# bevanda/Learning-Based-MPC

Hardware: AMD Instinct MI355X
Metric: QP-steps/s (whole node) at N=20 Moore-Greitzer; KKT-residual vs MATLAB ref (higher is better)
Workload: dtype f64; 1 GPU; C2: MG LMPC (F1) N=20, 616-row terminal set, batch 1024 per GPU, fp64; batch_per_gpu=1024, horizon=20, parallelism=dp1, streams=1

## Files before the change

### learning-based-mpc_amd/csrc/bqp_ocp.hip

```cpp
#include <hip/hip_runtime.h>
#include <math.h>
#include <stdint.h>
#include <stdlib.h>

#include <type_traits>

#include "bqp_internal.h"
#include "bqp_lanes.h"
#include "bqp_wave.h"

namespace bqp {

#ifdef BQP_F32
typedef float real;
typedef float2 real2;
#define BQP_SFX _f32
namespace sp {
#else
typedef double real;
typedef double2 real2;
#define BQP_SFX
namespace dp {
#endif
#define BQP_CAT2(a, b) a##b
#define BQP_CAT(a, b) BQP_CAT2(a, b)

#define WAVE 64
#ifdef BQP_F32
#define BQP_LNG_OK 0
#else
#define BQP_LNG_OK 1
#endif
#ifdef BQP_F32
#define PIV_FLOOR 1e-7
#else
#define PIV_FLOOR 1e-14
#endif
#define MU_BLOWUP 1e6
#ifdef BQP_F32
#define FEAS_GUARD 1e-6
#define BQP_POLISH 0
#else
#define FEAS_GUARD 1e-8
#define BQP_POLISH 1
#endif
#ifndef BQP_EXP_NOROW
#define BQP_EXP_NOROW 0
#endif
#ifndef BQP_EXP_NOSTAGE
#define BQP_EXP_NOSTAGE 0
#endif
#define TAU_FAST_AFF 0.99
#define TAU_FAST_MU 1e-6
#define TAU_FAST 0.99999
#define TAU_FAST_END 0.99999
#define TAU_FAST_MIN 0.995
#define CMAX_K 100.0
#define SOC_ALPHA 0.1
#define DEG_POLISH 1e-10
#define POL_RHO 2e6
#define POL_ROUNDS 8
#define POL_PASS 3
#define POL_CG 40
#define POL_CG_SING 1e-2
#define POL_STAG 0.5

__device__ __forceinline__ double frcp(double t) {
    double r = __builtin_amdgcn_rcp(t);
    double e = __builtin_fma(-t, r, 1.0);
    r = __builtin_fma(r, e, r);
    e = __builtin_fma(-t, r, 1.0);
    return __builtin_fma(r, e, r);
}
__device__ __forceinline__ float frcp(float t) {
    float r = __builtin_amdgcn_rcpf(t);
    return __builtin_fmaf(r, __builtin_fmaf(-t, r, 1.0f), r);
}

__device__ __forceinline__ int opq(int v) {
    asm volatile("" : "+v"(v));
    return v;
}
__device__ __forceinline__ int opq_s(int v) {
    asm volatile("" : "+s"(v));
    return v;
}

__device__ __forceinline__ double fmar(double a, double b, double c) { return __builtin_fma(a, b, c); }
__device__ __forceinline__ float fmar(float a, float b, float c) { return __builtin_fmaf(a, b, c); }
constexpr bool SWEEP_DPP_FMAC = sizeof(real) == 8;
#ifndef BQP_SWEEP_ROWS
#define BQP_SWEEP_ROWS 1
#endif
#ifdef BQP_F32
#define MADD(acc, a, b) acc = fmar((a), (b), (acc))
#else
#define MADD(acc, a, b) acc += (a) * (b)
#endif

template <int N>
__device__ __forceinline__ bool chol_small(const real (&M)[N][N], real (&L)[N][N]) {
    bool ok = true;
    real d0 = M[0][0];
    if (!(d0 > PIV_FLOOR * M[0][0])) d0 = PIV_FLOOR * M[0][0];
    ok = ok && (d0 > 0.0);
    if constexpr (N == 2) {
        const real r0 = frcp(d0);
        const real l10 = M[1][0] * r0;
        real d1 = M[1][1] - l10 * M[1][0];
        if (!(d1 > PIV_FLOOR * M[1][1])) d1 = PIV_FLOOR * M[1][1];
        ok = ok && (d1 > 0.0);
        L[0][0] = r0;
        L[0][1] = 0.0;
        L[1][0] = l10;
        L[1][1] = frcp(d1);
    } else {
        L[0][0] = sqrt(d0);
    }
    return ok;
}
template <int N>
__device__ __forceinline__ void chol_solve_small(const real* L, real (&b)[N]) {
    if constexpr (N == 2) {
        const real w1 = (b[1] - L[2] * b[0]) * L[3];
        b[0] = b[0] * L[0] - L[2] * w1;
        b[1] = w1;
    } else {
        b[0] = b[0] * L[0];
    }
}

__host__ __device__ constexpr int pk_len(int NS) { return NS * (NS + 1) / 2; }
__host__ __device__ constexpr int pk_stride(int NS) {
    return (((pk_len(NS) + 1) & ~1) % 4 == 0) ? ((pk_len(NS) + 1) & ~1) + 2 : ((pk_len(NS) + 1) & ~1);
}
__host__ __device__ constexpr int pk_idx(int NS, int i, int j) {
    return i <= j ? i * NS - i * (i - 1) / 2 + (j - i) : j * NS - j * (j - 1) / 2 + (i - j);
}

__host__ __device__ constexpr int stg_len(int NX, int NU) { return NX * NX + NX * NU + NX; }
__host__ __device__ constexpr int stg_stride(int NX, int NU) { return stg_len(NX, NU) | 1; }

enum : int {
    X_CNT = 0,
    X_BSR,
    X_FEASB,
    X_CS,
    X_STOP,
    X_ALPHA,
    X_CMAX,
    X_FEASOK,
    X_FLAG,
    X_RHO,
    X_TF,
    X_DEG,
    X_PVA,
    X_PVIOL,
    X_PLNEG,
    X_PLMX,
    X_PCHG,
    X_PDEC,
    X_CGD,
    X_NXCH = 20
};
constexpr int X_NEXT = X_PVA;
static_assert(X_PVIOL == X_PVA + 1, "X_NEXT + 1 must be a polish-only slot");
constexpr int X_RSS = X_PLNEG;
constexpr int X_PEN = X_PLMX;

struct QpLds {
    int P, K, Lr, L0, AB, xs, xu, qt_xpi, rs, ru, re, pv, wv, bw, qu, fv, dsv, duv, dsc, duc, Dx, FD,
        blam, ebox, bnd, gpp, gpe, prp, hp, rp, xch, Fi, Hi, total;
    __host__ __device__ __forceinline__ static QpLds make(int N, int NX, int NU, int NP, int mpad, bool fpi = false,
                                          bool lng = false, bool hpsh = false, bool bndsh = false,
                                          bool hinst = false, bool stg = false) {
// ... 10 lines not shown
        o.qt_xpi = c; c += (N + 1) * NS;
        o.rs = c;     c += (N + 1) * NS;
        o.ru = c;     c += (N + 1) * NU;
        o.re = c;     c += lng ? 0 : (N + 1) * NS;
        o.pv = c;     c += (N + 1) * NS;
        o.wv = c;     c += (N + 1) * NS;
        o.bw = c;     c += (N + 1) * NU;
        o.qu = c;     c += (N + 1) * NU;
        if (lng) {
            o.fv = o.qt_xpi;
        } else {
            o.fv = c; c += (N + 1) * NS;
        }
        o.dsv = c;    c += (N + 1) * NS;
        o.duv = c;    c += (N + 1) * NU;
        o.dsc = c;    c += (N + 1) * NS;
        o.duc = c;    c += (N + 1) * NU;
        o.Dx = c;     c += (N + 1) * NV;
        o.FD = c;     c += NV * NV;
        o.blam = c;   c += (N + 1) * NB * (lng ? 1 : 2);
        o.ebox = c;   c += (N + 1) * NB * (lng ? 1 : 2);
        o.bnd = c;    c += bndsh ? 0 : (N + 1) * NB * 2;
        o.gpp = c;    c += NV;
        o.gpe = c;    c += NV;
        o.prp = c;    c += mpad;
        o.hp = c;     c += hpsh ? 0 : mpad;
        o.rp = c;     c += lng ? 0 : mpad;
        o.xch = c;    c += X_NXCH;
        o.Fi = c;     c += fpi ? NV * mpad : 0;
        o.Hi = c;     c += (hinst && !lng) ? (N + 1) * (NV * NV + 1) : 0;
        o.total = (c + 1) & ~1;
        return o;
    }
};

__host__ __device__ constexpr int hand_stage_w(int NS, int NU) { return 2 * NS + NU; }
__host__ __device__ constexpr int hand_rows_off(int N, int NS, int NU) {
    return ((N + 1) * hand_stage_w(NS, NU) + 63) & ~63;
}
#ifdef BQP_F32
#define BQP_HAND_IN 0
#define BQP_HAND_OUT 1
#else
#define BQP_HAND_IN 1
#define BQP_HAND_OUT 0
#endif
template <bool LONG, bool POL>
__device__ __forceinline__ bool hand_warm(const OcpKernelArgs& a, int inst) {
    return BQP_HAND_IN && LONG && a.hand_in && (a.hand_flag[inst] == 1 || a.hand_flag[inst] == 0) &&
           !(POL && a.pol_need[inst] == 2);
}

#ifdef BQP_STAMPS
#define STAMP(id)                                                          \
    do {                                                                   \
        __builtin_amdgcn_s_waitcnt(0);                                     \
        const unsigned long long _t = __builtin_amdgcn_s_memtime();        \
        st_acc[id] += _t - st_last;                                        \
        st_last = _t;                                                      \
    } while (0)
#define STAMP_DECL                                                         \
    unsigned long long st_last = __builtin_amdgcn_s_memtime();             \
    unsigned long long st_acc[16];                                         \
    _Pragma("unroll") for (int i_ = 0; i_ < 16; ++i_) st_acc[i_] = 0
#define STAMP_STORE(base)                                                  \
    do {                                                                   \
        if (lane == 0 && a.stamps) {                                       \
            _Pragma("unroll") for (int i_ = 0; i_ < 16; ++i_)              \
                a.stamps[(int64_t)inst * 32 + (base) + i_] = (double)st_acc[i_]; \
        }                                                                  \
    } while (0)
#elif defined(BQP_ISA_ONLY_MG10) || defined(BQP_ISA_ONLY_DI) || defined(BQP_ISA_ONLY_MG_LNG)
#define STAMP(id) asm volatile(";BQP_PHASE " #id)
#define STAMP_DECL do { } while (0)
#define STAMP_STORE(base) do { } while (0)
#else
#define STAMP(id) do { } while (0)
#define STAMP_DECL do { } while (0)
#define STAMP_STORE(base) do { } while (0)
#endif

#if defined(BQP_STAMPS) && defined(BQP_STAMPS_SPLIT)
#define STAMP_SPLIT(id) STAMP(id)
#else
#define STAMP_SPLIT(id) do { } while (0)
#endif

#define BARRIER() __syncthreads()
#define ROW_FENCE(q) do { if ((q) & 1) __builtin_amdgcn_sched_barrier(0); } while (0)

template <int NX, int NU, int NP, int SPL, bool POL, int G, bool STG = false, bool SOFT = false>
__device__ __forceinline__ void stage_wave(const OcpKernelArgs& a, real* W, const QpLds& L,
                                           const real* Hs, int lane_w, int inst, int pslot) {
    const int lane = lane_w;
    constexpr bool PC = POL && BQP_POLISH && !BQP_EXP_NOSTAGE;
    constexpr int NS = NX + NP;
    constexpr int NV = NS + NU;
    constexpr int NB = NX + NU;
    static_assert(G == 1 || (SPL == 1 && lanes::compiled(NS, NU, G)), "lane groups: short horizons only");
    static_assert(!STG || (G == 1 && sizeof(real) == 8), "per-stage models: fp64, G = 1");
    static_assert(!STG || SWEEP_DPP_FMAC, "per-stage models: the sweeps' DPP form only");
    static_assert(!SOFT || (STG && !POL), "soft state bounds: per-stage-model solve kernels only");
    constexpr int ES = lanes::entries_per_lane(NS, G);
    const int N = a.N, kp = a.kp, hstride = a.hstride;
    auto stage_of = [&](int ln, int j) __attribute__((always_inline)) -> int {
        if constexpr (G > 1) return lanes::stage_lane(ln, N, G).k;
        else return ln + WAVE * j;
    };
    real* X = W + L.xch;
    STAMP_DECL;
    constexpr bool LNG = BQP_LNG_OK && SPL == 2;
#define BQP_HK(k) const real* Hk = Hs + (k) * hstride; \
    const double* Hkg = (a.H_inst ? a.H_inst + (int64_t)inst * (N + 1) * hstride : a.H) + (int64_t)(k) * hstride
#define BQP_HV(idx) (LNG ? (real)Hkg[idx] : Hk[idx])
    real* Pgl = LNG ? (real*)a.Pg + (int64_t)pslot * (N + 1) * pk_stride(NS) : nullptr;
    if (!LNG && a.H_inst) {
        real* Hl = W + L.Hi;
        const double* Hg = a.H_inst + (int64_t)inst * (N + 1) * hstride;
        for (int i = lane; i < (N + 1) * hstride; i += WAVE) Hl[i] = (real)Hg[i];
        wave_sync();
        Hs = Hl;
    }

    const double* Ag = STG ? a.A + (int64_t)inst * a.sA : nullptr;
    const double* Bg = STG ? a.B + (int64_t)inst * a.sB : nullptr;
    const double* cg = (STG && a.c) ? a.c + (int64_t)inst * a.sc : nullptr;
    constexpr int MW = stg_len(NX, NU), MST = stg_stride(NX, NU);
    if constexpr (STG) {
        if constexpr (!LNG) {
            for (int t = lane; t < N * MW; t += WAVE) {
                const int k = t / MW, e = t - k * MW;
                int kg = k;
                if constexpr (SOFT) { if (a.one_model) kg = 0; }
                real v;
                if (e < NX * NX) v = Ag[(int64_t)kg * (NX * NX) + e];
                else if (e < NX * NX + NX * NU) v = Bg[(int64_t)kg * (NX * NU) + (e - NX * NX)];
                else v = cg ? cg[(int64_t)kg * NX + (e - NX * NX - NX * NU)] : 0.0;
                W[L.AB + k * MST + e] = v;
            }
        }
    } else {
        const double* A = a.A + (int64_t)inst * a.sA;
        const double* B = a.B + (int64_t)inst * a.sB;
        if (lane < NS * NS) {
            const int i = lane / NS, j = lane % NS;
            W[L.AB + lane] = (i < NX && j < NX) ? A[j * NX + i] : (i == j ? 1.0 : 0.0);
        }
        if (lane < NS * NU) {
            const int i = lane / NU, j = lane % NU;
            W[L.AB + NS * NS + lane] = (i < NX) ? B[j * NX + i] : 0.0;
        }
        if (lane < NS) W[L.AB + NS * NS + NS * NU + lane] = (lane < NX && a.c) ? a.c[(int64_t)inst * a.sc + lane] : 0.0;
    }
    wave_sync();
    auto mdl = [&](int k, int e) __attribute__((always_inline)) -> real {
        const int km = k < N ? k : N - 1;
        if constexpr (LNG) {
            int kg = km;
            if constexpr (SOFT) { if (a.one_model) kg = 0; }
            if (e < NX * NX) return (real)Ag[(int64_t)kg * (NX * NX) + e];
            if (e < NX * NX + NX * NU) return (real)Bg[(int64_t)kg * (NX * NU) + (e - NX * NX)];
            return cg ? (real)cg[(int64_t)kg * NX + (e - NX * NX - NX * NU)] : real(0);
        } else {
            return W[L.AB + km * MST + e];
        }
    };
    auto Abar = [&](int k, int i, int j) __attribute__((always_inline)) -> real {
        if constexpr (STG) {
// ... 159 lines not shown
#pragma unroll
                    for (int c = 0; c < NS; ++c) MADD(acc, Abar(k, i, c), s[j][c]);
#pragma unroll
                    for (int c = 0; c < NU; ++c) MADD(acc, Bbar(k, i, c), u[j][c]);
                    if constexpr (!LNG) W[L.re + k * NS + i] = acc;
                    fe = fmax(fe, fabs(acc));
                }
            }
        }
        feasA = wmax(fe);
        gsA = wmax(gs);
    };

    bool rez = false;
    auto re_at = [&](int j, int k, int i) __attribute__((always_inline)) -> real {
        if constexpr (PC) { if (rez) return real(0); }
        real acc = cb(k, i) - W[L.xs + (k + 1) * NS + i];
#pragma unroll
        for (int c = 0; c < NS; ++c) MADD(acc, Abar(k, i, c), s[j][c]);
#pragma unroll
        for (int c = 0; c < NU; ++c) MADD(acc, Bbar(k, i, c), u[j][c]);
        return acc;
    };

    auto combine = [&]() __attribute__((always_inline)) -> real {
        const int lane = opq(lane_w);
        real gpp[NV];
#pragma unroll
        for (int c = 0; c < NV; ++c) gpp[c] = W[L.gpp + c];
        real st = 0;
#pragma unroll
        for (int j = 0; j < SPL; ++j) {
            const int k = stage_of(lane, j);
            if (k > N) continue;
            real r[NS], ru[NU];
#pragma unroll
            for (int i = 0; i < NS; ++i) r[i] = W[L.rs + k * NS + i];
#pragma unroll
            for (int i = 0; i < NU; ++i) ru[i] = W[L.ru + k * NU + i];
#pragma unroll
            for (int i = 0; i < NX; ++i) {
                if constexpr (LNG) {
                    r[i] += W[L.blam + k * NB + i];
                } else {
                    r[i] += W[L.blam + (k * NB + i) * 2];
                    r[i] -= W[L.blam + (k * NB + i) * 2 + 1];
                }
            }
#pragma unroll
            for (int i = 0; i < NU; ++i) {
                if constexpr (LNG) {
                    ru[i] += W[L.blam + k * NB + NX + i];
                } else {
                    ru[i] += W[L.blam + (k * NB + NX + i) * 2];
                    ru[i] -= W[L.blam + (k * NB + NX + i) * 2 + 1];
                }
            }
            if (k == kp) {
#pragma unroll
                for (int i = 0; i < NS; ++i) r[i] += gpp[i];
                if (kp < N) {
#pragma unroll
                    for (int i = 0; i < NU; ++i) ru[i] += gpp[NS + i];
                }
            }
            if (k == 0) {
#pragma unroll
                for (int i = 0; i < NX; ++i) r[i] = 0.0;
            }
#pragma unroll
            for (int i = 0; i < NS; ++i) { st = fmax(st, fabs(r[i])); W[L.rs + k * NS + i] = r[i]; }
#pragma unroll
            for (int i = 0; i < NU; ++i) { st = fmax(st, fabs(ru[i])); W[L.ru + k * NU + i] = ru[i]; }
        }
        wave_sync();
        return wmax(st);
    };

    constexpr int PST = pk_stride(NS);
    constexpr int NPK = pk_len(NS);
    constexpr int NUT = NU * (NU + 1) / 2;
    constexpr int VAL = 1 + 2 * NU + NUT;
    constexpr int VPL = (VAL + 3) / 4;
    static_assert(4 * NPK <= WAVE, "one quad per packed entry of P");
    const int fq = lane >> 2, fql = lane & 3;
    const bool fquad = fq < NPK;
    int ie = 0, je = 0;
    {
        int e = 0;
#pragma unroll
        for (int i = 0; i < NS; ++i)
#pragma unroll
            for (int j = i; j < NS; ++j, ++e)
                if (e == fq) { ie = i; je = j; }
    }
    auto vrc = [&](int v, int& r, int& c) __attribute__((always_inline)) {
        if (v == 0) { r = ie; c = je; }
        else if (v <= NU) { r = ie; c = NS + v - 1; }
        else if (v <= 2 * NU) { r = je; c = NS + v - NU - 1; }
        else {
            int t = v - 2 * NU - 1, x = 0;
#pragma unroll
            for (int xx = 0; xx < NU; ++xx) if (t >= NU - xx) { t -= NU - xx; x = xx + 1; } else break;
            r = NS + x; c = NS + x + t;
        }
    };
    real cf[STG ? 1 : VPL][STG ? 1 : NPK];
    int vr[VPL], vc[VPL];
    int fr[VPL], fc[VPL];
#pragma unroll
    for (int t = 0; t < VPL; ++t) {
        const int v = fql + 4 * t;
        int r = 0, c = 0;
        if (v < VAL) vrc(v, r, c);
        vr[t] = r; vc[t] = c;
        if constexpr (STG) {
            fr[t] = r < NX ? r * NX : (r >= NS ? (NX + r - NS) * NX : -1);
            fc[t] = c < NX ? c * NX : (c >= NS ? (NX + c - NS) * NX : -1);
        } else {
            auto Fab = [&](int a_, int r_) __attribute__((always_inline)) -> real {
                return r_ < NS ? Abar(0, a_, r_) : Bbar(0, a_, r_ - NS);
            };
            int m = 0;
#pragma unroll
            for (int a_ = 0; a_ < NS; ++a_)
#pragma unroll
                for (int b = a_; b < NS; ++b, ++m) {
                    real x = Fab(a_, r) * Fab(b, c);
                    if (a_ != b) x = fmar(Fab(b, r), Fab(a_, c), x);
                    cf[t][m] = (v < VAL) ? x : real(0);
                }
        }
    }
    struct HNoModel {};
    struct HModel { real mr[VPL][NX], mc[VPL][NX]; };
    struct HRaw : std::conditional_t<STG, HModel, HNoModel> { real h[VPL], d[VPL]; };
    auto load_h = [&](int k, HRaw& o) __attribute__((always_inline)) {
        BQP_HK(k);
#pragma unroll
        for (int t = 0; t < VPL; ++t) {
            o.h[t] = BQP_HV(vr[t] * NV + vc[t]);
            o.d[t] = W[L.Dx + k * NV + vr[t]];
            if constexpr (STG) {
#pragma unroll
                for (int a_ = 0; a_ < NX; ++a_) {
                    const real xr = mdl(k, (fr[t] < 0 ? 0 : fr[t]) + a_);
                    const real xc = mdl(k, (fc[t] < 0 ? 0 : fc[t]) + a_);
                    o.mr[t][a_] = fr[t] < 0 ? real(0) : xr;
                    o.mc[t][a_] = fc[t] < 0 ? real(0) : xc;
                }
            }
        }
    };
    auto cf_at = [&](const HRaw& o, int t, int a_, int b) __attribute__((always_inline)) -> real {
        if constexpr (STG) {
            auto Fr = [&](int i) __attribute__((always_inline)) -> real {
                return i < NX ? o.mr[t][i < NX ? i : 0] : (vr[t] == i ? real(1) : real(0));
            };
            auto Fc = [&](int i) __attribute__((always_inline)) -> real {
                return i < NX ? o.mc[t][i < NX ? i : 0] : (vc[t] == i ? real(1) : real(0));
            };
            real x = Fr(a_) * Fc(b);
            if (a_ != b) x = fmar(Fr(b), Fc(a_), x);
            return (fql + 4 * t < VAL) ? x : real(0);
        } else {
            return real(0);
        }
    };
    auto ht = [&](int k, const HRaw& o, int t) __attribute__((always_inline)) -> real {
        real v = o.h[t] + (vr[t] == vc[t] ? o.d[t] : real(0));
        if (k == kp) v += W[L.FD + vr[t] * NV + vc[t]];
        return v;
    };
    real pu[PST];
    auto read_p = [&](int k) __attribute__((always_inline)) {
        wave_sync();
        const real2* src = reinterpret_cast<const real2*>(W + L.P + (LNG ? (k & 1) : k) * PST);
#pragma unroll
        for (int q = 0; q < PST / 2; ++q) {
            const real2 t2 = src[q];
            pu[2 * q] = t2.x;
            pu[2 * q + 1] = t2.y;
        }
    };
    auto Pm = [&](int a_, int b_) __attribute__((always_inline)) -> real { return pu[pk_idx(NS, a_, b_)]; };
    auto factor = [&]() __attribute__((always_inline)) -> bool {
        HRaw raw, nxt;
        {
            load_h(N, raw);
            const real v0 = ht(N, raw, 0);
            if (fquad && fql == 0) {
                W[L.P + (LNG ? (N & 1) : N) * PST + fq] = v0;
                if constexpr (LNG) Pgl[N * PST + fq] = v0;
            }
        }
        read_p(N);
        bool ok = true;
        auto fstage = [&](int k, const HRaw& raw) __attribute__((always_inline)) {
            real mv[VPL];
#pragma unroll
            for (int t = 0; t < VPL; ++t) {
                real sp0 = 0, sp1 = 0, sp2 = 0, sp3 = 0;
                if constexpr (STG) {
                    int m = 0;
#pragma unroll
                    for (int a_ = 0; a_ < NS; ++a_)
#pragma unroll
                        for (int b = a_; b < NS; ++b, ++m) {
                            const real cm = cf_at(raw, t, a_, b);
                            if ((m & 3) == 0) sp0 = fmar(cm, pu[m], sp0);
                            if ((m & 3) == 1) sp1 = fmar(cm, pu[m], sp1);
                            if ((m & 3) == 2) sp2 = fmar(cm, pu[m], sp2);
                            if ((m & 3) == 3) sp3 = fmar(cm, pu[m], sp3);
                        }
                } else {
#pragma unroll
                for (int m = 0; m < NPK; ++m) {
                    if ((m & 3) == 0) sp0 = fmar(cf[t][m], pu[m], sp0);
                    if ((m & 3) == 1) sp1 = fmar(cf[t][m], pu[m], sp1);
                    if ((m & 3) == 2) sp2 = fmar(cf[t][m], pu[m], sp2);
                    if ((m & 3) == 3) sp3 = fmar(cf[t][m], pu[m], sp3);
                }
                }
                mv[t] = ht(k, raw, t) + ((sp0 + sp1) + (sp2 + sp3));
            }
            real g[VAL];
#pragma unroll
            for (int v = 0; v < VAL; ++v) {
                const int s = v & 3;
                const real src = mv[v >> 2];
                g[v] = (s == 0) ? dpp_mov0<0x00>(src)
                     : (s == 1) ? dpp_mov0<0x55>(src)
                     : (s == 2) ? dpp_mov0<0xAA>(src)
                                : dpp_mov0<0xFF>(src);
            }
            real pv, Kc[NU], Lf[NU * NU];
            if constexpr (NU == 1) {
                ok = ok && (g[3] > 0.0);
                const real rinv = frcp(g[3]);
                Lf[0] = rinv;
                pv = fmar(-(g[1] * rinv), g[2], g[0]);
                Kc[0] = -(g[2] * rinv);
            } else {
                real Mu[NU][NU], Lc[NU][NU];
                {
                    int t = 2 * NU + 1;
#pragma unroll
                    for (int x = 0; x < NU; ++x)
#pragma unroll
                        for (int y = x; y < NU; ++y, ++t) { Mu[x][y] = g[t]; Mu[y][x] = g[t]; }
                }
                ok = chol_small<NU>(Mu, Lc) && ok;
#pragma unroll
                for (int x = 0; x < NU; ++x)
#pragma unroll
                    for (int y = 0; y < NU; ++y) Lf[x * NU + y] = Lc[x][y];
                real y[NU];
#pragma unroll
                for (int x = 0; x < NU; ++x) y[x] = g[1 + NU + x];
                chol_solve_small<NU>(Lf, y);
                real acc = g[1] * y[0];
#pragma unroll
                for (int x = 1; x < NU; ++x) acc = fmar(g[1 + x], y[x], acc);
                pv = g[0] - acc;
#pragma unroll
                for (int x = 0; x < NU; ++x) Kc[x] = -y[x];
            }
            if (fquad && fql == 0) {
                W[L.P + (LNG ? (k & 1) : k) * PST + fq] = pv;
                if constexpr (LNG) Pgl[k * PST + fq] = pv;
                if (ie == je) {
#pragma unroll
                    for (int x = 0; x < NU; ++x) W[L.K + k * NU * NS + x * NS + je] = Kc[x];
                }
                if (fq == 0) {
#pragma unroll
                    for (int x = 0; x < NU * NU; ++x) W[L.Lr + k * NU * NU + x] = Lf[x];
                }
            }
            read_p(k);
        };
        if constexpr (LNG) {
            HRaw r0, r1, r2;
            load_h(N - 1, r0);
            if (N >= 2) load_h(N - 2, r1);
            for (int k = N - 1; k >= 0; k -= 3) {
                if (k >= 2) load_h(k - 2, r2);
                fstage(k, r0);
                if (k < 1) break;
                if (k >= 3) load_h(k - 3, r0);
                fstage(k - 1, r1);
                if (k < 2) break;
                if (k >= 4) load_h(k - 4, r1);
                fstage(k - 2, r2);
            }
        } else {
            load_h(N - 1, raw);
            for (int k = N - 1; k >= 0; --k) {
                if (k > 0) load_h(k - 1, nxt);
                fstage(k, raw);
                raw = nxt;
            }
        }
        real Pt[NP][NP], L0[NP][NP];
#pragma unroll
        for (int x = 0; x < NP; ++x)
#pragma unroll
            for (int y = 0; y < NP; ++y) Pt[x][y] = Pm(NX + x, NX + y);
        if constexpr (NP == 1) {
            ok = ok && (Pt[0][0] > 0.0);
            L0[0][0] = 1.0 / Pt[0][0];
        } else {
            ok = chol_small<NP>(Pt, L0) && ok;
        }
        if (lane == 0) {
#pragma unroll
            for (int x = 0; x < NP; ++x)
#pragma unroll
                for (int y = 0; y < NP; ++y) W[L.L0 + x * NP + y] = L0[x][y];
        }
        if constexpr (LNG) asm volatile("s_waitcnt vmcnt(0)" ::: "memory");
        wave_sync();
        return ok;
    };
    auto load_pk = [&](int k, real* pk) __attribute__((always_inline)) {
        if constexpr (LNG) {
            const real* src = Pgl + k * PST;
#pragma unroll
            for (int e = 0; e < NPK; ++e) pk[e] = __hip_atomic_load(src + e, __ATOMIC_RELAXED, __HIP_MEMORY_SCOPE_AGENT);
        } else {
#pragma unroll
            for (int e = 0; e < NPK; ++e) pk[e] = W[L.P + k * PST + e];
        }
    };

    auto prep_iter = [&]() __attribute__((always_inline)) {
        const int lane = opq(lane_w);
        if constexpr (G > 1) {
            const lanes::StageLane sl = lanes::stage_lane(lane, N, G);
            const int k = sl.k;
            if (k < N) {
                const real* Pn = W + L.P + (k + 1) * PST;
                const real* Kk = W + L.K + k * NU * NS;
                real rek[NS], wk[NS];
#pragma unroll
                for (int c = 0; c < NS; ++c) rek[c] = W[L.re + k * NS + c];
#pragma unroll
                for (int i = 0; i < NS; ++i) {
                    real v = 0.0;
#pragma unroll
                    for (int c = 0; c < NS; ++c) MADD(v, Pn[pk_idx(NS, i, c)], rek[c]);
                    wk[i] = v;
                }
#pragma unroll
                for (int x = 0; x < NU; ++x) {
                    real v = 0.0;
#pragma unroll
                    for (int c = 0; c < NS; ++c) MADD(v, Bbar(k, c, x), wk[c]);
                    W[L.bw + k * NU + x] = v;
                }
#pragma unroll
                for (int t = 0; t < ES; ++t) {
                    const int i = lanes::entry(NS, G, sl.g, t);
                    real v = 0.0;
#pragma unroll
                    for (int c = 0; c < NS; ++c) {
                        real ph = Abar(k, c, i);
#pragma unroll
                        for (int x = 0; x < NU; ++x) MADD(ph, Bbar(k, c, x), Kk[x * NS + i]);
                        MADD(v, ph, wk[c]);
                    }
                    W[L.wv + k * NS + i] = v;
                }
            }
            return;
        }
#pragma unroll
        for (int j = 0; j < SPL; ++j) {
            const int k = stage_of(lane, j);
            if (k < N) {
                real Pn_[LNG ? PST : 1];
                const real* Pn = W + L.P + (k + 1) * PST;
                if constexpr (LNG) { load_pk(k + 1, Pn_); Pn = Pn_; }
                const real* Kk = W + L.K + k * NU * NS;
                real rek[NS], wk[NS];
#pragma unroll
                for (int c = 0; c < NS; ++c) rek[c] = LNG ? re_at(j, k, c) : W[L.re + k * NS + c];
#pragma unroll
                for (int i = 0; i < NS; ++i) {
                    real v = 0.0;
#pragma unroll
// ... 597 lines not shown
            for (int i = 0; i < NS; ++i) MADD(s[j][i], al, dsk[i]);
            if (k < N) {
#pragma unroll
                for (int i = 0; i < NU; ++i) MADD(u[j][i], al, W[idu + k * NU + i]);
            }
        }
    };

    real feasA = 0, gsA = 0;
    real minv, bscale;
    int flag = 0, it0 = 0;
    if (hand_warm<SPL == 2, POL>(a, inst)) {
        const float* hb = a.hand_in + (int64_t)inst * a.hand_stride;
        constexpr int SW = hand_stage_w(NS, NU);
#pragma unroll
        for (int j = 0; j < SPL; ++j) {
            const int k = stage_of(lane, j);
            if (k > N) continue;
#pragma unroll
            for (int i = 0; i < NS; ++i) {
                s[j][i] = (k == 0 && i < NX) ? s[j][i] : (real)hb[k * SW + i];
                pi[j][i] = (real)hb[k * SW + NS + i];
            }
#pragma unroll
            for (int i = 0; i < NU; ++i) u[j][i] = (k < N) ? (real)hb[k * SW + 2 * NS + i] : 0.0;
        }
        write_state();
        stage_partials(feasA, gsA);
        BARRIER();
        minv = 1.0 / fmax(X[X_CNT], 1.0);
        bscale = fmax(x0max, X[X_BSR]);
        it0 = a.hand_it[inst];
    } else {
        write_state();
        stage_partials(feasA, gsA);
        BARRIER();
        minv = 1.0 / fmax(X[X_CNT], 1.0);
        bscale = fmax(x0max, X[X_BSR]);
        combine();
        if (!factor()) flag = -8;
        prep_iter();
        BARRIER();
        solve(L.dsv, L.duv);
        update_stage(1.0, L.dsv, L.duv);
        BARRIER();
        BARRIER();
        write_state();
        stage_partials(feasA, gsA);
    }

    int it = 0;
    real mu = 0.0, mu_min = INFINITY, stat = 0.0, feas = 0.0, feq = 0.0, fin = 0.0;
    const int max_iter = a.max_iter;
    for (it = 0;; ++it) {
        BARRIER();
        STAMP(0);
        stat = combine();
        if constexpr (SOFT) stat = fmax(stat, X[X_RSS]);
        STAMP(1);
        STAMP(2);
        feq = feasA;
        fin = X[X_FEASB];
        feas = fmax(feq, fin);
        mu = X[X_CS] * minv;
        bool stop = false;
        if (flag != 0) {
            stop = true;
        } else if (stat <= a.tol_stat * (1.0 + gsA) && feas <= a.tol_feas * (1.0 + bscale) &&
                   mu <= a.tol_comp && (!BQP_POLISH || X[X_CMAX] <= CMAX_K * a.tol_comp)) {
            flag = 1; stop = true;
#ifdef BQP_F32
        } else if (mu <= a.tol_comp && feas <= a.tol_feas * (1.0 + bscale) && isfinite(stat)) {
            flag = 1; stop = true;
#endif
        } else if (!(isfinite(stat) && isfinite(feas) && isfinite(mu))) {
            flag = -8; stop = true;
        } else if (mu > MU_BLOWUP * mu_min && feas > FEAS_GUARD * (1.0 + bscale)) {
            flag = -2; stop = true;
        } else {
            mu_min = fmin(mu_min, mu);
            if (it == max_iter) stop = true;
        }
        if (!stop && !factor()) { flag = -8; stop = true; }
        if (!stop) prep_iter();
        STAMP(3);
        if (lane == 0) {
            X[X_STOP] = stop ? 1.0 : 0.0;
            X[X_FEASOK] = (feas <= FEAS_GUARD * (1.0 + bscale)) ? 1.0 : 0.0;
            X[X_FLAG] = (real)flag;
            if constexpr (PC) {
                X[X_RHO] = POL_RHO * (1.0 + gsA);
                X[X_TF] = 1e-12 * (1.0 + bscale);
            }
        }
        BARRIER();
        STAMP(4);
        if (stop) break;
        solve(L.dsv, L.duv);
        STAMP(5);
        BARRIER();
        BARRIER();
        STAMP(6);
        solve(L.dsc, L.duc);
        STAMP(7);
        BARRIER();
        dual_dir(L.dsc);
        BARRIER();
        STAMP(8);
        const real al = X[X_ALPHA];
        update_stage_dir(al, L.dsc, L.duc);
        write_state();
        stage_partials(feasA, gsA);
        STAMP(9);
    }

    real polished = 0.0;
    bool pi_kept = false;
    if constexpr (PC) {
        BARRIER();
        const bool dopol = a.polish > 0 && flag != -2 &&
                           (flag != 1 || (a.polish > 1 && X[X_DEG] > DEG_POLISH)) && isfinite(gsA);
        if (dopol) {
            STAMP(15);
#pragma unroll
            for (int j = 0; j < SPL; ++j) {
                const int k = lane + WAVE * j;
                if (a.pi_out && k >= 1 && k <= N) {
                    double* po = a.pi_out + ((int64_t)inst * N + (k - 1)) * NX;
#pragma unroll
                    for (int i = 0; i < NX; ++i) po[i] = pi[j][i];
                }
                if (k <= N) {
#pragma unroll
                    for (int i = 0; i < NS; ++i) W[L.dsv + k * NS + i] = s[j][i];
#pragma unroll
                    for (int i = 0; i < NU; ++i) W[L.duv + k * NU + i] = (k < N) ? u[j][i] : 0.0;
                }
            }
            const real tf = 1e-12 * (1.0 + bscale);
            int rd = 0, pass = 0, m = 0, dec = 0;
            real pst = 0.0;
            auto zero_stage_res = [&]() __attribute__((always_inline)) {
#pragma unroll
                for (int j = 0; j < SPL; ++j) {
                    const int k = stage_of(lane, j);
                    if (k > N) continue;
#pragma unroll
                    for (int i = 0; i < NS; ++i) {
                        W[L.rs + k * NS + i] = 0.0;
                        if constexpr (!LNG) W[L.re + k * NS + i] = 0.0;
                    }
#pragma unroll
                    for (int i = 0; i < NU; ++i) W[L.ru + k * NU + i] = 0.0;
                }
                wave_sync();
            };
            for (;;) {
                stage_partials(feasA, gsA);
                BARRIER();
                BARRIER();
                pst = combine();
                const real va = X[X_PVA];
                if (m != 1) {
                    dec = factor() ? 0 : 3;
                    pass = 0;
                } else {
                    const bool pok = isfinite(pst) && pst <= a.tol_stat * (1.0 + gsA) && va <= tf;
                    if (!pok && pass + 1 < POL_PASS) {
// ... 1871 lines not shown
```

### learning-based-mpc_amd/csrc/bqp_wave.h

```cpp
#pragma once
#include <hip/hip_runtime.h>
#include <math.h>

namespace bqp {

__device__ __forceinline__ void wave_sync() {
    __builtin_amdgcn_fence(__ATOMIC_RELEASE, "wavefront");
    __builtin_amdgcn_wave_barrier();
    __builtin_amdgcn_fence(__ATOMIC_ACQUIRE, "wavefront");
}

template <int CTRL, int ROWM>
__device__ __forceinline__ double dpp_mov(double old, double v) {
    const int2 o = __builtin_bit_cast(int2, old);
    const int2 x = __builtin_bit_cast(int2, v);
    int2 r;
    r.x = __builtin_amdgcn_update_dpp(o.x, x.x, CTRL, ROWM, 0xf, false);
    r.y = __builtin_amdgcn_update_dpp(o.y, x.y, CTRL, ROWM, 0xf, false);
    return __builtin_bit_cast(double, r);
}
template <int CTRL>
__device__ __forceinline__ double dpp_mov0(double v) {
    const int2 x = __builtin_bit_cast(int2, v);
    int2 r;
// ... 84 lines not shown
    v += dpp_mov<0x143, 0xc>(0.0f, v);
    return lane63(v);
}
__device__ __forceinline__ float wmax(float v) {
    v = fmaxf(v, dpp_mov<0xB1, 0xf>(-INFINITY, v));
    v = fmaxf(v, dpp_mov<0x4E, 0xf>(-INFINITY, v));
    v = fmaxf(v, dpp_mov<0x141, 0xf>(-INFINITY, v));
    v = fmaxf(v, dpp_mov<0x140, 0xf>(-INFINITY, v));
    v = fmaxf(v, dpp_mov<0x142, 0xa>(-INFINITY, v));
    v = fmaxf(v, dpp_mov<0x143, 0xc>(-INFINITY, v));
    return lane63(v);
}
__device__ __forceinline__ float wmin(float v) { return -wmax(-v); }
__device__ __forceinline__ float rl(float v, int src) {
    return __builtin_bit_cast(float, __builtin_amdgcn_readlane(__builtin_bit_cast(int, v), src));
}

template <int C>
__device__ __forceinline__ double rbc(double v) {
    return __builtin_amdgcn_update_dpp(0.0, v, 0x150 + C, 0xf, 0xf, true);
}
template <int C>
__device__ __forceinline__ float rbc(float v) {
    return __builtin_bit_cast(float, __builtin_amdgcn_update_dpp(0, __builtin_bit_cast(int, v),
                                                                 0x150 + C, 0xf, 0xf, true));
}
template <int Q>
__device__ __forceinline__ double xrow_bcast(double v) {
    double a = v, b = v;
    pl16_swap(a, b);
    double c = (Q & 1) ? b : a, d = c;
    pl32_swap(c, d);
    return (Q >> 1) ? d : c;
}

template <int C, int NC, typename T>
__device__ __forceinline__ void rbc_all(T v, T (&p)[NC]) {
    p[C] = rbc<C>(v);
    if constexpr (C + 1 < NC) rbc_all<C + 1, NC>(v, p);
}

template <int C, bool FRESH = false, typename T>
__device__ __forceinline__ void fmac_rbc(T& acc, T v, T ph) {
    static_assert(sizeof(T) == 8, "fmac_rbc: fp64 only (the fp32 sweeps keep rbc + plain products)");
    static_assert(C >= 0 && C < 16, "fmac_rbc: lane of a 16-lane row");
    if constexpr (FRESH)
        asm("s_nop 1\n\t"
            "v_fmac_f64_dpp %0, %1, %2 row_newbcast:%3 row_mask:0xf bank_mask:0xf bound_ctrl:1"
            : "+v"(acc) : "v"(v), "v"(ph), "n"(C));
    else
        asm("v_fmac_f64_dpp %0, %1, %2 row_newbcast:%3 row_mask:0xf bank_mask:0xf bound_ctrl:1"
            : "+v"(acc) : "v"(v), "v"(ph), "n"(C));
}
template <int C, int NC, typename T>
__device__ __forceinline__ void fmac_rbc_seq(T& acc, T v, const T (&ph)[NC]) {
    fmac_rbc<C, C == 0>(acc, v, ph[C]);
    if constexpr (C + 1 < NC) fmac_rbc_seq<C + 1, NC>(acc, v, ph);
}
#define BQP_FMAC_RBC(OP, C) \
    "v_fmac_f64_dpp %0, %2, %" #OP " row_newbcast:" #C " row_mask:0xf bank_mask:0xf bound_ctrl:1\n\t"
#define BQP_CHAIN_HEAD \
    "v_mov_b64 %0, %1\n\t" \
    "s_nop 0\n\t"
template <int NC, typename T>
__device__ __forceinline__ T fmac_rbc_chain(T q, T v, const T (&ph)[NC]) {
    static_assert(sizeof(T) == 8, "fmac_rbc_chain: fp64 only");
    T acc;
    if constexpr (NC == 4) {
        asm(BQP_CHAIN_HEAD BQP_FMAC_RBC(3, 0) BQP_FMAC_RBC(4, 1) BQP_FMAC_RBC(5, 2) BQP_FMAC_RBC(6, 3)
            : "=&v"(acc) : "v"(q), "v"(v), "v"(ph[0]), "v"(ph[1]), "v"(ph[2]), "v"(ph[3]));
    } else if constexpr (NC == 5) {
        asm(BQP_CHAIN_HEAD BQP_FMAC_RBC(3, 0) BQP_FMAC_RBC(4, 1) BQP_FMAC_RBC(5, 2) BQP_FMAC_RBC(6, 3)
            BQP_FMAC_RBC(7, 4)
            : "=&v"(acc) : "v"(q), "v"(v), "v"(ph[0]), "v"(ph[1]), "v"(ph[2]), "v"(ph[3]), "v"(ph[4]));
    } else {
        acc = q;
        fmac_rbc_seq<0, NC>(acc, v, ph);
    }
    return acc;
}
#undef BQP_CHAIN_HEAD
#undef BQP_FMAC_RBC

template <int CTRL, typename T, int KI, int KO>
__device__ __forceinline__ void tsum_step(const T (&in)[KI], T (&out)[KO], bool hi) {
#pragma unroll
    for (int p = 0; p < KO; ++p) {
        const T a = in[2 * p];
        const T b = (2 * p + 1 < KI) ? in[2 * p + 1] : T(0);
        const T keep = hi ? b : a;
        const T send = hi ? a : b;
        out[p] = keep + dpp_mov0<CTRL>(send);
    }
}
template <typename T, int K>
__device__ __forceinline__ T wsum_t(const T (&v)[K], int lane) {
    static_assert(K >= 2 && K <= 32, "wsum_t: 2..32 values");
    constexpr int K1 = (K + 1) / 2, K2 = (K1 + 1) / 2, K3 = (K2 + 1) / 2, K4 = (K3 + 1) / 2;
    T w1[K1], w2[K2], w3[K3], w4[K4];
    tsum_step<0xB1>(v, w1, (lane & 1) != 0);
    tsum_step<0x4E>(w1, w2, (lane & 2) != 0);
    tsum_step<0x124>(w2, w3, (lane & 4) != 0);
    tsum_step<0x128>(w3, w4, (lane & 8) != 0);
    T a = w4[0], b = T(0);
    if constexpr (K4 > 1) b = w4[K4 - 1];
    pl16_swap(a, b);
    T c = a + b, d = c;
    pl32_swap(c, d);
    return c + d;
}

}
```

Before: 2.808 million QP-steps/s.

## Factor Riccati stage with row-layout packed P held in registers via DPP broadcasts

Remaps the factor's lane assignment so each 16-lane row holds one packed entry of P per lane, with the four rows carrying different value groups. The P-times-coefficient dot product now uses v_fmac_f64_dpp row_newbcast from the register-resident P, and results are gathered with permlane swaps. This removes the LDS write/read round trip of P at each stage along with its wave syncs. It also inlines the 2x2 Cholesky solve and moves a timing stamp. The new path is limited to fp64, SPL==1 and NPK<=16, and relies on inline asm and permlane ops that must be correct for this layout.

```diff
diff --git a/learning-based-mpc_amd/csrc/bqp_ocp.hip b/learning-based-mpc_amd/csrc/bqp_ocp.hip
--- a/learning-based-mpc_amd/csrc/bqp_ocp.hip
+++ b/learning-based-mpc_amd/csrc/bqp_ocp.hip
@@ -91,6 +91,9 @@
 constexpr bool SWEEP_DPP_FMAC = sizeof(real) == 8;
 #ifndef BQP_SWEEP_ROWS
 #define BQP_SWEEP_ROWS 1
+#endif
+#ifndef BQP_FACTOR_ROWS
+#define BQP_FACTOR_ROWS 1
 #endif
 #ifdef BQP_F32
 #define MADD(acc, a, b) acc = fmar((a), (b), (acc))
@@ -267,8 +270,10 @@
 
 #if defined(BQP_STAMPS) && defined(BQP_STAMPS_SPLIT)
 #define STAMP_SPLIT(id) STAMP(id)
+#define STAMP_PLAIN(id) do { } while (0)
 #else
 #define STAMP_SPLIT(id) do { } while (0)
+#define STAMP_PLAIN(id) STAMP(id)
 #endif
 
 #define BARRIER() __syncthreads()
@@ -594,8 +599,12 @@
     constexpr int NUT = NU * (NU + 1) / 2;
     constexpr int VAL = 1 + 2 * NU + NUT;
     constexpr int VPL = (VAL + 3) / 4;
+    constexpr bool FACTOR_ROWS = BQP_FACTOR_ROWS && sizeof(real) == 8 && SPL == 1;
     static_assert(4 * NPK <= WAVE, "one quad per packed entry of P");
-    const int fq = lane >> 2, fql = lane & 3;
+    static_assert(!FACTOR_ROWS || NPK <= 16, "FACTOR_ROWS: one packed entry of P per lane of a row");
+    static_assert(!FACTOR_ROWS || NP <= 2, "FACTOR_ROWS: the theta block's entries are taken one by one");
+    const int fq = FACTOR_ROWS ? ((lane & 15) < NPK ? (lane & 15) : NPK - 1) : lane >> 2;
+    const int fql = FACTOR_ROWS ? lane >> 4 : lane & 3;
     const bool fquad = fq < NPK;
     int ie = 0, je = 0;
     {
@@ -698,22 +707,42 @@
     auto Pm = [&](int a_, int b_) __attribute__((always_inline)) -> real { return pu[pk_idx(NS, a_, b_)]; };
     auto factor = [&]() __attribute__((always_inline)) -> bool {
         HRaw raw, nxt;
+        real pl = 0;
         {
             load_h(N, raw);
             const real v0 = ht(N, raw, 0);
+            if constexpr (FACTOR_ROWS) {
+                pl = xrow_bcast<0>(v0);
+                W[L.P + N * PST + fq] = pl;
+            } else {
             if (fquad && fql == 0) {
                 W[L.P + (LNG ? (N & 1) : N) * PST + fq] = v0;
                 if constexpr (LNG) Pgl[N * PST + fq] = v0;
             }
-        }
-        read_p(N);
+            }
+        }
+        if constexpr (!FACTOR_ROWS) read_p(N);
         bool ok = true;
         auto fstage = [&](int k, const HRaw& raw) __attribute__((always_inline)) {
             real mv[VPL];
 #pragma unroll
             for (int t = 0; t < VPL; ++t) {
                 real sp0 = 0, sp1 = 0, sp2 = 0, sp3 = 0;
-                if constexpr (STG) {
+                if constexpr (FACTOR_ROWS) {
+                    real sp[4];
+                    if constexpr (STG) {
+                        real cm[NPK];
+                        int m = 0;
+#pragma unroll
+                        for (int a_ = 0; a_ < NS; ++a_)
+#pragma unroll
+                            for (int b = a_; b < NS; ++b, ++m) cm[m] = cf_at(raw, t, a_, b);
+                        fmac_rbc_dot4(sp, pl, cm);
+                    } else {
+                        fmac_rbc_dot4(sp, pl, cf[t]);
+                    }
+                    sp0 = sp[0]; sp1 = sp[1]; sp2 = sp[2]; sp3 = sp[3];
+                } else if constexpr (STG) {
                     int m = 0;
 #pragma unroll
                     for (int a_ = 0; a_ < NS; ++a_)
@@ -737,6 +766,15 @@
                 mv[t] = ht(k, raw, t) + ((sp0 + sp1) + (sp2 + sp3));
             }
             real g[VAL];
+            if constexpr (FACTOR_ROWS) {
+#pragma unroll
+                for (int t = 0; t < VPL; ++t) {
+                    real g4[4];
+                    xrow_gather(mv[t], g4);
+#pragma unroll
+                    for (int s = 0; s < 4; ++s) if (4 * t + s < VAL) g[4 * t + s] = g4[s];
+                }
+            } else {
 #pragma unroll
             for (int v = 0; v < VAL; ++v) {
                 const int s = v & 3;
@@ -745,6 +783,7 @@
                      : (s == 1) ? dpp_mov0<0x55>(src)
                      : (s == 2) ? dpp_mov0<0xAA>(src)
                                 : dpp_mov0<0xFF>(src);
+            }
             }
             real pv, Kc[NU], Lf[NU * NU];
             if constexpr (NU == 1) {
@@ -770,13 +809,28 @@
                 real y[NU];
 #pragma unroll
                 for (int x = 0; x < NU; ++x) y[x] = g[1 + NU + x];
-                chol_solve_small<NU>(Lf, y);
+                if constexpr (FACTOR_ROWS && NU == 2) {
+                    const real w1 = (y[1] - Lf[2] * y[0]) * Lf[3];
+                    y[0] = fmar(y[0], Lf[0], -(Lf[2] * w1));
+                    y[1] = w1;
+                } else {
+                    chol_solve_small<NU>(Lf, y);
+                }
                 real acc = g[1] * y[0];
 #pragma unroll
                 for (int x = 1; x < NU; ++x) acc = fmar(g[1 + x], y[x], acc);
                 pv = g[0] - acc;
 #pragma unroll
                 for (int x = 0; x < NU; ++x) Kc[x] = -y[x];
+            }
+            if constexpr (FACTOR_ROWS) {
+                W[L.P + k * PST + fq] = pv;
+#pragma unroll
+                for (int x = 0; x < NU; ++x) W[L.K + k * NU * NS + x * NS + je] = Kc[x];
+#pragma unroll
+                for (int x = 0; x < NU * NU; ++x) W[L.Lr + k * NU * NU + x] = Lf[x];
+                pl = pv;
+                return;
             }
             if (fquad && fql == 0) {
                 W[L.P + (LNG ? (k & 1) : k) * PST + fq] = pv;
@@ -818,7 +872,14 @@
 #pragma unroll
         for (int x = 0; x < NP; ++x)
 #pragma unroll
-            for (int y = 0; y < NP; ++y) Pt[x][y] = Pm(NX + x, NX + y);
+            for (int y = 0; y < NP; ++y) Pt[x][y] = FACTOR_ROWS ? real(0) : Pm(NX + x, NX + y);
+        if constexpr (FACTOR_ROWS) {
+            Pt[0][0] = rbc<pk_idx(NS, NX, NX)>(pl);
+            if constexpr (NP == 2) {
+                Pt[0][1] = Pt[1][0] = rbc<pk_idx(NS, NX, NX + 1)>(pl);
+                Pt[1][1] = rbc<pk_idx(NS, NX + 1, NX + 1)>(pl);
+            }
+        }
         if constexpr (NP == 1) {
             ok = ok && (Pt[0][0] > 0.0);
             L0[0][0] = 1.0 / Pt[0][0];
@@ -1582,8 +1643,9 @@
             if (it == max_iter) stop = true;
         }
         if (!stop && !factor()) { flag = -8; stop = true; }
+        STAMP_SPLIT(3);
         if (!stop) prep_iter();
-        STAMP(3);
+        STAMP_PLAIN(3);
         if (lane == 0) {
             X[X_STOP] = stop ? 1.0 : 0.0;
             X[X_FEASOK] = (feas <= FEAS_GUARD * (1.0 + bscale)) ? 1.0 : 0.0;
diff --git a/learning-based-mpc_amd/csrc/bqp_wave.h b/learning-based-mpc_amd/csrc/bqp_wave.h
--- a/learning-based-mpc_amd/csrc/bqp_wave.h
+++ b/learning-based-mpc_amd/csrc/bqp_wave.h
@@ -190,6 +190,55 @@
 #undef BQP_CHAIN_HEAD
 #undef BQP_FMAC_RBC
 
+#define BQP_DOT4_ZERO \
+    "v_mov_b64 %0, 0\n\tv_mov_b64 %1, 0\n\tv_mov_b64 %2, 0\n\tv_mov_b64 %3, 0\n\t"
+#define BQP_DOT4_FMAC(ACC, OP, C) \
+    "v_fmac_f64_dpp %" #ACC ", %4, %" #OP " row_newbcast:" #C " row_mask:0xf bank_mask:0xf bound_ctrl:1\n\t"
+template <int M, int NC, typename T>
+__device__ __forceinline__ void fmac_rbc_dot4_seq(T (&s)[4], T v, const T (&c)[NC]) {
+    fmac_rbc<M, (M < 4)>(s[M & 3], v, c[M]);
+    if constexpr (M + 1 < NC) fmac_rbc_dot4_seq<M + 1, NC>(s, v, c);
+}
+template <int NC, typename T>
+__device__ __forceinline__ void fmac_rbc_dot4(T (&s)[4], T v, const T (&c)[NC]) {
+    static_assert(sizeof(T) == 8, "fmac_rbc_dot4: fp64 only");
+    static_assert(NC >= 4 && NC <= 16, "fmac_rbc_dot4: one entry per lane of a 16-lane row");
+    if constexpr (NC == 10) {
+        asm(BQP_DOT4_ZERO
+            BQP_DOT4_FMAC(0, 5, 0) BQP_DOT4_FMAC(1, 6, 1) BQP_DOT4_FMAC(2, 7, 2) BQP_DOT4_FMAC(3, 8, 3)
+            BQP_DOT4_FMAC(0, 9, 4) BQP_DOT4_FMAC(1, 10, 5) BQP_DOT4_FMAC(2, 11, 6) BQP_DOT4_FMAC(3, 12, 7)
+            BQP_DOT4_FMAC(0, 13, 8) BQP_DOT4_FMAC(1, 14, 9)
+            : "=&v"(s[0]), "=&v"(s[1]), "=&v"(s[2]), "=&v"(s[3])
+            : "v"(v), "v"(c[0]), "v"(c[1]), "v"(c[2]), "v"(c[3]), "v"(c[4]), "v"(c[5]), "v"(c[6]),
+              "v"(c[7]), "v"(c[8]), "v"(c[9]));
+    } else if constexpr (NC == 15) {
+        asm(BQP_DOT4_ZERO
+            BQP_DOT4_FMAC(0, 5, 0) BQP_DOT4_FMAC(1, 6, 1) BQP_DOT4_FMAC(2, 7, 2) BQP_DOT4_FMAC(3, 8, 3)
+            BQP_DOT4_FMAC(0, 9, 4) BQP_DOT4_FMAC(1, 10, 5) BQP_DOT4_FMAC(2, 11, 6) BQP_DOT4_FMAC(3, 12, 7)
+            BQP_DOT4_FMAC(0, 13, 8) BQP_DOT4_FMAC(1, 14, 9) BQP_DOT4_FMAC(2, 15, 10) BQP_DOT4_FMAC(3, 16, 11)
+            BQP_DOT4_FMAC(0, 17, 12) BQP_DOT4_FMAC(1, 18, 13) BQP_DOT4_FMAC(2, 19, 14)
+            : "=&v"(s[0]), "=&v"(s[1]), "=&v"(s[2]), "=&v"(s[3])
+            : "v"(v), "v"(c[0]), "v"(c[1]), "v"(c[2]), "v"(c[3]), "v"(c[4]), "v"(c[5]), "v"(c[6]),
+              "v"(c[7]), "v"(c[8]), "v"(c[9]), "v"(c[10]), "v"(c[11]), "v"(c[12]), "v"(c[13]),
+              "v"(c[14]));
+    } else {
+        s[0] = s[1] = s[2] = s[3] = T(0);
+        fmac_rbc_dot4_seq<0, NC>(s, v, c);
+    }
+}
+#undef BQP_DOT4_FMAC
+#undef BQP_DOT4_ZERO
+
+template <typename T>
+__device__ __forceinline__ void xrow_gather(T v, T (&g)[4]) {
+    T a = v, b = v;
+    pl16_swap(a, b);
+    g[0] = a; g[2] = a;
+    pl32_swap(g[0], g[2]);
+    g[1] = b; g[3] = b;
+    pl32_swap(g[1], g[3]);
+}
+
 template <int CTRL, typename T, int KI, int KO>
 __device__ __forceinline__ void tsum_step(const T (&in)[KI], T (&out)[KO], bool hi) {
 #pragma unroll
```

After: 2.920 million QP-steps/s, median of 6. +4.0%, better.
